# aldma/Bazinga.jl

Hardware: AMD Instinct MI355X
Metric: PANOC inner iterations/sec, n=10^7 l1-quadratic (higher is better)
Workload: dtype f64

## Files before the change

### bazinga.jl_amd/csrc/bz_kernels.h

```cpp
#pragma once
#include <algorithm>
#include <type_traits>

#include <hip/hip_runtime.h>
#include <stdint.h>
#include <math.h>

#include "../../include/bazinga_hip.h"

namespace bz {

constexpr int BLOCK   = 256;
constexpr int WAVES   = BLOCK / 64;
constexpr int PSTRIDE = 2048;

struct ScalarSrc {
    const double* p;
    int count;
    int stride;
};

template <class T> struct PackN;
template <> struct PackN<double> { static constexpr int N = 2; };
template <> struct PackN<float>  { static constexpr int N = 4; };
// ... 2006 lines not shown
                acc[10] = mul_acc(s, nr, acc[10]);
                acc[11] = mul_acc(yy, nr, acc[11]);
            }
        }
        st(x_d, i0, cnt, pxd);
        st(z, i0, cnt, pz);
        st(res, i0, cnt, pr);
        st(s_new, i0, cnt, ps);
        st(y_new, i0, cnt, py);
        if (gx_out) st(gx_out, i0, cnt, pg1);
        if (gz_out) st(gz_out, i0, cnt, pg2);
    });
    block_reduce_store<12>(acc, 1u << 9, parts, slot0);
}

template <class T, int MM> struct CompactVecs {
    const T* S[MM];
    const T* Y[MM];
    int m;
};
struct GateRec {
    unsigned long long w[32];
    unsigned long long seq;
    double val[13];
};
constexpr unsigned long long GATE_ABORT = 1ull << 63;
constexpr unsigned GATE_SPIN_HOST = 2500000u, GATE_SPIN_DEV = 60000000u;

template <int MM> struct CompactCoef {
    double u1[MM];
    double u2h[MM];
    double H0;
    double gam0;
    int uni_rt, trial_rt;
    unsigned long long gate_seq;
    const GateRec* gate_host;
    GateRec* gate_dev;
    int* gate_timeout;
    unsigned gate_spin_host, gate_spin_dev;
};

template <class T, int MM>
__global__ void __launch_bounds__(BLOCK)
k_gram_dots(CompactVecs<T, MM> V, const T* __restrict__ res, int64_t n, double* __restrict__ parts,
            int slot0) {
    double acc[2 * MM];
#pragma unroll
    for (int k = 0; k < 2 * MM; ++k) acc[k] = 0.0;
    bz_for_chunks<T>(n, [&](const int64_t i0, const auto cnt_) {
        const int cnt = cnt_;
        Pack<T> pr = ld(res, i0, cnt);
#pragma unroll
        for (int i = 0; i < MM; ++i) {
            if (i < V.m) {
                Pack<T> ps = ld(V.S[i], i0, cnt), py = ld(V.Y[i], i0, cnt);
#pragma unroll
                for (int e = 0; e < PackN<T>::N; ++e)
                    if (e < cnt) {
                        const T v = T(-1) * pr.v[e];
                        acc[i] = mul_acc(ps.v[e], v, acc[i]);
                        acc[MM + i] = mul_acc(py.v[e], v, acc[MM + i]);
                    }
            }
        }
    });
    block_reduce_store<2 * MM>(acc, 0u, parts, slot0);
// ... 587 lines not shown
                        if ((sq & ~GATE_ABORT) == C.gate_seq) break;
                        __builtin_amdgcn_s_sleep(2);
                        if (++spins > C.gate_spin_dev) { sq = C.gate_seq | GATE_ABORT; *C.gate_timeout = 7; break; }
                    }
                }
                if (lane == 0) gate_sh = sq;
            }
            __syncthreads();
            if (gate_sh & GATE_ABORT) return false;
#pragma unroll
            for (int i = 0; i < MM; ++i) {
                u1[i] = (T)__hip_atomic_load(&C.gate_dev->val[i], __ATOMIC_RELAXED, __HIP_MEMORY_SCOPE_AGENT);
                u2h[i] = (T)__hip_atomic_load(&C.gate_dev->val[5 + i], __ATOMIC_RELAXED, __HIP_MEMORY_SCOPE_AGENT);
            }
            H0 = (T)__hip_atomic_load(&C.gate_dev->val[10], __ATOMIC_RELAXED, __HIP_MEMORY_SCOPE_AGENT);
            z = (T*)(uintptr_t)__double_as_longlong(__hip_atomic_load(&C.gate_dev->val[11], __ATOMIC_RELAXED, __HIP_MEMORY_SCOPE_AGENT));
        }
        }
        return true;
    };
    static_assert(XR == 0 || XR == 2, "XR: stored pairs (0) or iterates with re-evaluated residuals (2)");
    static_assert(XR != 2 || (SPEC && OFF32), "the iterate-history form is pipelined");
    if (SPEC && !OFF32) {
#pragma unroll
        for (int i = 0; i < MM; ++i) { asm volatile("" : "+v"(u1[i])); asm volatile("" : "+v"(u2h[i])); }
        asm volatile("" : "+v"(H0));
        asm volatile("" : "+v"(gl));
        asm volatile("" : "+v"(gamma));
    }
    constexpr bool UDIV = XR == 2 && sizeof(T) == 8;
    T rmu_u = T(0), rgam = T(0);
    if constexpr (UDIV) { rgam = T(1) / gamma; if (uni >= 1) rmu_u = T(1) / P.mu_uniform; }
    const T gam0 = (T)C.gam0, gl0 = gam0 * P.g_lambda;
    constexpr int NS = 10 + 4 * MM + 2;
    double acc[NS];
#pragma unroll
    for (int k = 0; k < NS; ++k) acc[k] = 0.0;
    constexpr bool PIPE = SPEC && OFF32 && XR == 2;
    constexpr int NSTREAMS = MM + 1 + (fam_fk(FAM) ? 2 : 0) + (UNI >= 2 ? 0 : (UNI == 1 ? 1 : 2)) + (TRIAL == 0 ? 0 : 1) +
                             (GKC == FAM_G_L1BOX ? 1 : 0) + (GKC == FAM_G_INDBOX_VEC ? 2 : 0) + (DKC == FAM_D_BOX_VEC ? 2 : 0);
    constexpr int DEPTH = NSTREAMS <= 11 ? 2 : 1;
    constexpr bool NTP = NT && PP == 0;
    struct Stage { Pack<T> q, b, mu, muy, px, ps[MM], xt, gu, glo, ghi, dlo, dhi; };
    using PolQB = std::integral_constant<bool, NTP>;
    using PolNT = std::integral_constant<bool, NT>;
    auto for_fixed_streams = [&](Stage& S, auto&& f) {
        if (fk == BZ_F_DIAG_QUADRATIC) { f(S.q, P.q, PolQB{}); f(S.b, P.b, PolQB{}); }
        if (uni < 1) f(S.mu, P.mu, PolNT{});
        if (uni < 2) f(S.muy, P.muy, PolNT{});
        f(S.px, x, PolNT{});
        if (trial) f(S.xt, (const T*)x_d, PolNT{});
#pragma unroll
        for (int i = 0; i < MM; ++i) f(S.ps[i], V.S[i], PolNT{});
    };
    auto load_stage = [&](Stage& S, unsigned bo) {
        asm volatile("" : "+v"(bo));
        for_fixed_streams(S, [&](Pack<T>& d, const T* p, auto pol) { d = ldo<T, decltype(pol)::value>(p, bo); });
        if constexpr (GKC == FAM_G_L1BOX) S.gu = ldo<T, NT>(P.g_u, bo);
        if constexpr (GKC == FAM_G_INDBOX_VEC) {
            S.glo = P.g_lo_vec ? ldo<T, NT>(P.g_lo_vec, bo) : splat(P.g_lo);
            S.ghi = P.g_hi_vec ? ldo<T, NT>(P.g_hi_vec, bo) : splat(P.g_hi);
        }
        if constexpr (DKC == FAM_D_BOX_VEC) {
            S.dlo = P.D_lo_vec ? ldo<T, NT>(P.D_lo_vec, bo) : splat(P.D_lo);
            S.dhi = P.D_hi_vec ? ldo<T, NT>(P.D_hi_vec, bo) : splat(P.D_hi);
        }
// ... 32 lines not shown
            for (int i = 0; i < MM; ++i) {
                ps[i] = ldo<T, NT>(V.S[i], bo);
                py[i] = ldo<T, NT>(V.Y[i], bo);
            }
        } else {
            if (SPEC && !FAMILY) {
                L.q = ldp<T, NTP>(P.q, i0, cnt); L.b = ldp<T, NTP>(P.b, i0, cnt);
                if (P.uni >= 1) L.mu = splat(P.mu_uniform); else L.mu = ldp<T, NT>(P.mu, i0, cnt);
                if (P.uni >= 2) L.muy = splat(T(0)); else L.muy = ldp<T, NT>(P.muy, i0, cnt);
                L.dlo = splat(P.D_lo); L.dhi = splat(P.D_hi);
                L.gu = splat(T(0)); L.glo = splat(T(0)); L.ghi = splat(T(0));
            } else {
                load_params<T, NT>(P, i0, cnt, L, true, true, true);
                if (FAMILY && uni >= 1) L.mu = splat(P.mu_uniform);
                if (FAMILY && uni >= 2) L.muy = splat(T(0));
            }
            px = ldp<T, NT>(x, i0, cnt);
            if constexpr (XR != 2) prp = ldp<T, NT>(res_prev, i0, cnt);
#pragma unroll
            for (int i = 0; i < MM; ++i)
                if (i < m) {
                    ps[i] = ldp<T, NT>(V.S[i], i0, cnt);
                    if constexpr (XR != 2) py[i] = ldp<T, NT>(V.Y[i], i0, cnt);
                }
        }
        if constexpr (XR == 2) {
            Pack<T> rr[MM + 1];
#pragma unroll
            for (int e = 0; e < N; ++e) {
                if constexpr (UDIV) rmu.v[e] = (uni >= 1) ? rmu_u : T(1) / L.mu.v[e];
#pragma unroll
                for (int i = 0; i <= MM; ++i) {
                    T zz;
                    const T gi = (i == 0) ? gam0 : gamma;
                    const T gli = (i == 0) ? gl0 : gl;
                    rr[i].v[e] = resid_elem<T>(fk, dk, gk, (i < MM) ? ps[i].v[e] : px.v[e], L, e, gi, gli, zz, UDIV,
                                               rmu.v[e], (i < MM) ? ps[i].v[e ^ 1] : px.v[e ^ 1]);
                }
            }
            prp = rr[MM];
#pragma unroll
            for (int i = 0; i < MM; ++i)
#pragma unroll
                for (int e = 0; e < N; ++e) {
                    const T nx = (i + 1 < MM) ? ps[i + 1].v[e] : px.v[e];
                    ps[i].v[e] = nx - ps[i].v[e];
                    py[i].v[e] = rr[i + 1].v[e] - rr[i].v[e];
                }
        }
        if (!trial) compact_d<T, MM>(m, H0, u1, u2h, prp, ps, py, d);
        Pack<T> pxd, pz, pr, pss, pyy, pg1, pgt;
#pragma unroll
        for (int e = 0; e < N; ++e) pxd.v[e] = trial ? pxt.v[e] : px.v[e] + d.v[e];
        T f1[N], p1[N];
#pragma unroll
        for (int e = 0; e < N; ++e) {
            const T xd = pxd.v[e];
            ALOut<T> o1 = al_elem(fk, dk, xd, L.q.v[e], L.b.v[e], L.mu.v[e], L.muy.v[e], L.dlo.v[e], L.dhi.v[e],
                                  pxd.v[e ^ 1] + L.muy.v[e ^ 1], e & 1, UDIV, rmu.v[e]);
            T t = gamma * o1.grad;
            T y = xd - t;
            T zz = prox_elem(gk, y, gl, L.gu.v[e], L.glo.v[e], L.ghi.v[e], pgt.v[e]);
            pz.v[e] = zz; pr.v[e] = xd - zz;
            pg1.v[e] = o1.grad; f1[e] = o1.fterm; p1[e] = o1.pterm;
        }
#pragma unroll
        for (int e = 0; e < N; ++e) {
            const T xd = pxd.v[e], zz = pz.v[e], r = pr.v[e];
            ALOut<T> o2 = al_elem(fk, dk, zz, L.q.v[e], L.b.v[e], L.mu.v[e], L.muy.v[e], L.dlo.v[e], L.dhi.v[e],
                                  pz.v[e ^ 1] + L.muy.v[e ^ 1], e & 1, UDIV, rmu.v[e]);
            T sv = xd - px.v[e];
            T yy = r - prp.v[e];
            T w = UDIV ? div_u(r, gamma, rgam) : r / gamma;
// ... 769 lines not shown
```

### bazinga.jl_amd/csrc/bz_solver.hip

```cpp
#include "bz_solver.h"
#include "bz_spmv.h"
#include "bz_als_dense.h"
#include "bz_csr_host.h"

#include <hip/hip_ext.h>

#include <algorithm>
#include <array>
#include <atomic>
#include <chrono>
#include <cmath>
#include <cstdio>
#include <cstdlib>
#include <cstring>
#include <limits>
#include <optional>
#include <tuple>
#include <type_traits>

namespace bz {

Ctx::~Ctx() {
    for (int r = 0; r < P2P_MAXRANKS; ++r)
        if (mbox_opened[r] && mbox_peer[r]) (void)hipIpcCloseMemHandle(mbox_peer[r]);
// ... 67 lines not shown
    PersistTimeout() : Error(BZ_ERR_HIP, "persistent two-loop kernel: grid barrier timed out (blocks not co-resident?)") {}
};

bool& callback_abort_flag() {
    static thread_local bool flag = false;
    return flag;
}

enum Cat : int { C_TWOLOOP = 0, C_FUSED = 1, C_ALGRAD = 2, C_FB = 3, C_UPDATE = 4,
                 C_COLLECT = 5, C_GATHER = 6, C_MISC = 7, C_DOT = 8, C_GEMV = 9, C_PERSIST = 10, C_GEMV_MFMA = 11, C_FUSED_IT = 12,
                 C_STENCIL_FB = 13, C_STENCIL_UPD = 14, C_XD = 15 };

static int env_int(const char* name, int dflt) { const char* e = std::getenv(name); return e ? std::atoi(e) : dflt; }
static long long env_ll(const char* name, long long dflt) { const char* e = std::getenv(name); return e ? std::atoll(e) : dflt; }
static std::optional<int> env_opt(const char* name) { const char* e = std::getenv(name); return e ? std::optional<int>(std::atoi(e)) : std::nullopt; }
struct CreateKnobs {
    std::optional<int> grid = env_opt("BZ_GRID");
    std::optional<int> persist_blocks = env_opt("BZ_PERSIST_BLOCKS");
    int dense_fused = env_int("BZ_DENSE_FUSED", 1);
    std::optional<int> dense_kp = env_opt("BZ_DENSE_KP");
    std::optional<int> spmv_l = env_opt("BZ_SPMV_L");
    int spq_fused = env_int("BZ_SPQ_FUSED", 1);
    int spls_fused = env_int("BZ_SPLS_FUSED", 1);
    int test_dense_timeout = env_int("BZ_TEST_DENSE_TIMEOUT", 0);
    unsigned dense_spin = (unsigned)env_ll("BZ_DENSE_SPIN", 0);
};
struct BeginKnobs {
    explicit BeginKnobs(int nranks) : gate(env_int("BZ_GATE", nranks > 1 ? 0 : 1)) {}
    int gate;
    int xr = env_int("BZ_XR", 2);
    int skipz = env_int("BZ_SKIPZ", 1);
    int gfc = env_int("BZ_GFC", 0);
    int trialfuse = env_int("BZ_TRIALFUSE", 1);
    int fused_begin = env_int("BZ_FUSED_BEGIN", 1);
    int slackfast = env_int("BZ_SLACKFAST", 1);
    int slackkind = env_int("BZ_SLACKKIND", 1);
    int suc_grid = env_int("BZ_SUC_GRID", 1);
    int stencil_regx = env_int("BZ_STENCIL_REGX", 1);
    int affine_blend = env_int("BZ_AFFINE_BLEND", 1);
    int densesmall = env_int("BZ_DENSESMALL", 1);
    int nt = env_int("BZ_NT", -1);
    int keepp = env_int("BZ_KEEPP", -1);
    int ldsq = env_int("BZ_LDSQ", -1);
    int famrt = env_int("BZ_FAMRT", 0);
    int spec = env_int("BZ_SPEC", 1);
    int xdnt = env_int("BZ_XDNT", 1);
    bool gemv_valu = std::getenv("BZ_GEMV_VALU") != nullptr;
    long long persist_min_n = env_ll("BZ_PERSIST_MIN_N", 300000);
    bool test_persist_timeout = env_int("BZ_TEST_PERSIST_TIMEOUT", 0) != 0;
    int test_gate_timeout = env_int("BZ_TEST_GATE_TIMEOUT", 0);
    unsigned gate_spin = (unsigned)env_ll("BZ_GATE_SPIN", 0);
};
static int read_uni_knob() { return env_int("BZ_UNI", 2); }

template <class F> static void with_bool(bool b, F&& f) { if (b) f(std::true_type{}); else f(std::false_type{}); }
template <class F> static void with_uni(int u, F&& f) {
    if (u >= 2) f(std::integral_constant<int, 2>{});
    else if (u == 1) f(std::integral_constant<int, 1>{});
    else f(std::integral_constant<int, 0>{});
}

template <class T> class Solver final : public SolverBase {
   public:
    Solver(Ctx* c, const bz_problem_desc& d)
        : ctx(c), desc(d), n(d.n), ny(d.ny), nx(d.n), slack(d.slack != 0), env_(c->nranks) {
        if (n <= 0 || ny < 0) throw Error(BZ_ERR_ARG, "n must be positive");
// ... 820 lines not shown
        const T* yv = Y_[state_.lbfgs.spare].p;
        gemv_rows(HB_.p, n, n, yv, (const T*)nullptr, BHy_.p);
        gemv_cols(HB_.p, n, n, sv, b_rpc_, b_nch_, GT_.p, npad);
        {
            ElemParams<T> Pz = P;
            Pz.f_kind = BZ_F_ZERO;
            launch(C_MISC, k_gemv_t_finish<T>, grid, (const T*)GT_.p, b_nch_, npad, sv, Pz, BsH_.p, n, parts_.p, (int)SL_SCRATCH);
        }
        launch(C_MISC, k_dot<T>, grid, (const T*)BHy_.p, sv, T(1), n, parts_.p, (int)SL_AUX);
        launch(C_MISC, k_dot<T>, grid, sv, sv, T(1), n, parts_.p, (int)SL_AUX + 1);
        slot_n[SL_AUX] = slot_n[SL_AUX + 1] = grid;
        gather(SL_AUX, 2, 0u);
        auto v = collect({SL_AUX, SL_AUX + 1}, 0u);
        const T hys = T(v[0]), ss = T(v[1]);
        if (!(ss > T(0))) return;
        const T delta = hys / ss;
        T theta = T(1);
        if (std::abs(delta) < broyden_theta_bar_) {
            const T sg = delta >= T(0) ? T(1) : T(-1);
            theta = (T(1) - sg * broyden_theta_bar_) / (T(1) - delta);
        }
        const T denom = (T(1) / theta - T(1)) * ss + hys;
        if (denom == T(0) || denom != denom) return;
        launch(C_MISC, k_rank1_update<T>, (int)std::min<int64_t>(PSTRIDE, (n * n + BLOCK - 1) / BLOCK), HB_.p, sv,
               (const T*)BHy_.p, (const T*)BsH_.p, T(1) / denom, n);
    }
    bool compact_ok = false;

    struct GatePlan {
        const T* S[CM];
        const T* x;
        T* xd;
        double gam0, gamma;
        int uni, gfc, fam, m_now;
        bool nt, table, keep_params, lds_ring;
        auto key() const { return std::tie(x, xd, gam0, gamma, uni, gfc, fam, m_now, nt, table, keep_params, lds_ring); }
        bool operator==(const GatePlan& o) const { return std::equal(S, S + CM, o.S) && key() == o.key(); }
    };
    static constexpr double KEEP_PARAMS_BYTES = 256e6;
    bool keep_params(bool nt, bool table, int fam) const {
        if (!nt || table || fam != FAM_HEADLINE) return false;
        return env_.keepp >= 0 ? env_.keepp != 0 : (double)n * sizeof(T) * 2 <= KEEP_PARAMS_BYTES;
    }
    bool lds_ring(bool nt, bool table) const { return sizeof(T) == 8 && nt && !table && env_.ldsq != 0; }
    GateRec* gate_host_ = nullptr;
    GateRec* gate_host_dev_ = nullptr;
    DBuf<GateRec> gate_dev_;
    unsigned long long gate_seq_ = 0;
    bool gate_pending_ = false, more_coming_ = false;
    int gate_env_ = 1;
    bool gate_broken_ = false;
    int gate_sabotage_ = 0;
    int64_t n_gate_fallbacks_ = 0;
    GatePlan gate_plan_{};
    double gate_bytes_ = 0.0;
    int64_t n_gated_ = 0, n_gate_aborts_ = 0;
    void gate_alloc() {
        if (gate_host_) return;
        BZ_HIP(hipHostMalloc((void**)&gate_host_, sizeof(GateRec), hipHostMallocMapped));
        std::memset(gate_host_, 0, sizeof(GateRec));
        BZ_HIP(hipHostGetDevicePointer((void**)&gate_host_dev_, gate_host_, 0));
        gate_dev_.alloc(1);
    }
    bool small_vectors() const { return (double)vcap * sizeof(T) < 4.0e9; }
    int xr2_streams(int m_now) const { return (m_now + 1) + pstreams(true, true, true) + 1; }
    bool xr2_plan(int xc_, int m_now, const double* gring, int xr_run, bool zstore, GatePlan& pl) const {
        const int fam = fused_family();
        if (!(env_.xr && small_vectors() && fam >= 0 && xr_run >= m_now)) return false;
        for (int i = 1; i < m_now; ++i)
            if (gring[(xc_ - m_now + i + NXR) % NXR] != (double)state_.gamma) return false;
        std::memset(&pl, 0, sizeof(pl));
        for (int i = 0; i < CM; ++i) {
            const int slot = (xc_ - std::max(0, m_now - i) + NXR) % NXR;
            pl.S[i] = X_[slot].p;
            if (i == 0) pl.gam0 = gring[slot];
        }
        pl.x = X_[xc_].p; pl.xd = X_[(xc_ + 1) % NXR].p;
        pl.gamma = (double)state_.gamma; pl.uni = uni_; pl.fam = fam; pl.m_now = m_now;
        pl.gfc = env_.gfc > 0 ? std::min(grid, env_.gfc * std::max(1, num_cus)) : std::min(grid, std::max(1, num_cus));
        pl.nt = env_.nt >= 0 ? env_.nt != 0 : (double)n * sizeof(T) * (xr2_streams(m_now) + (zstore ? 1 : 0)) > 340e6;
        pl.table = !(env_.spec && fam == FAM_HEADLINE) || env_.famrt;
        pl.keep_params = keep_params(pl.nt, pl.table, fam);
        pl.lds_ring = lds_ring(pl.nt, pl.table);
        return true;
    }
    void launch_xr2(const GatePlan& pl, CompactCoef<CM> C, int trial, T* xd, T* zarg, T* resarg) {
        CompactVecs<T, CM> XV;
        XV.m = CM;
        for (int i = 0; i < CM; ++i) { XV.S[i] = pl.S[i]; XV.Y[i] = nullptr; }
        C.gam0 = pl.gam0;
        const T gam = (T)pl.gamma;
        auto go = [&](auto kernel) {
            launch(C_FUSED_IT, kernel, pl.gfc, XV, C, pl.x, (const T*)nullptr, P, gam, xd, zarg, resarg, (T*)nullptr,
                   (T*)nullptr, n, parts_.p, (int)SL_TRIAL);
        };
        if (pl.table) {
            C.uni_rt = pl.uni; C.trial_rt = trial;
            FusedFn<T> fn = (trial == 0 && !env_.famrt) ? family_kernel<T>(pl.fam, pl.nt, pl.uni) : nullptr;
            const bool ct = fn != nullptr;
            if (!fn) fn = family_kernel<T>(pl.fam, pl.nt, -1);
            if (!fn) throw Error(BZ_ERR_STATE, "no one-pass kernel instantiation for this oracle family");
            form_[C_FUSED_IT] = std::string("k_fused_compact<XR=2,UNI=") + (ct ? std::to_string(pl.uni) : std::string("-1")) + ",NT=" +
                                std::to_string(pl.nt ? 1 : 0) + ",TRIAL=" + (ct ? "0" : "-1") + ",FAM=" + std::to_string(pl.fam) + ">";
            go(fn);
            return;
        }
        form_[C_FUSED_IT] = std::string("k_fused_compact<XR=2,UNI=") + char('0' + pl.uni) + (pl.nt ? ",NT=1" : ",NT=0") +
                            (trial ? ",TRIAL=1" : ",TRIAL=0") + (pl.keep_params ? ",PP=1" : "") + (pl.lds_ring ? ",LQ=1>" : ">");
        with_bool(trial != 0, [&](auto tr) {
            with_uni(pl.uni, [&](auto un) {
                constexpr int TR = decltype(tr)::value, UNI = decltype(un)::value;
                if (pl.lds_ring) {
                    if constexpr (sizeof(T) == 8) {
                        if (pl.keep_params) go(k_fused_compact<T, CM, true, true, true, 2, UNI, TR, FAM_HEADLINE, 1, 1>);
                        else go(k_fused_compact<T, CM, true, true, true, 2, UNI, TR, FAM_HEADLINE, 0, 1>);
                    }
                } else if (pl.nt && pl.keep_params) go(k_fused_compact<T, CM, true, true, true, 2, UNI, TR, FAM_HEADLINE, 1>);
                else if (pl.nt) go(k_fused_compact<T, CM, true, true, true, 2, UNI, TR, FAM_HEADLINE, 0>);
                else go(k_fused_compact<T, CM, false, true, true, 2, UNI, TR, FAM_HEADLINE, 0>);
            });
        });
    }
    void gate_prelaunch(int xd, int m_now) {
        double gr[NXR];
        for (int i = 0; i < NXR; ++i) gr[i] = gring_[i];
        gr[xd] = (double)state_.gamma;
        GatePlan pl;
        if (!xr2_plan(xd, std::min(m_now + 1, state_.lbfgs.M), gr, xr_run_ + 1, false, pl)) return;
        gate_alloc();
        CompactCoef<CM> C2;
        std::memset(&C2, 0, sizeof(C2));
        C2.gate_spin_host = env_.gate_spin ? env_.gate_spin : GATE_SPIN_HOST;
        C2.gate_spin_dev = env_.gate_spin ? 8u * env_.gate_spin : GATE_SPIN_DEV;
        C2.gate_seq = ++gate_seq_; C2.gate_host = gate_host_dev_; C2.gate_dev = gate_dev_.p; C2.gate_timeout = ptimeout_dev_;
        mv(xr2_streams(pl.m_now));
        gate_bytes_ = pending_bytes_;
        launch_xr2(pl, C2, 0, pl.xd, (T*)nullptr, (T*)nullptr);
        gate_plan_ = pl; gate_pending_ = true;
    }
    void gate_release(const CompactCoef<CM>& C, T* zstore) {
        if (gate_sabotage_ > 0 && --gate_sabotage_ == 0) {
// ... 267 lines not shown
        if (!handles) throw Error(BZ_ERR_ARG, "null handles");
        BZ_HIP(hipSetDevice(ctx->device));
        for (int r = 0; r < ctx->nranks; ++r) {
            if (r == ctx->rank) { ar_peer_[r] = ar_local_; continue; }
            if (ar_peer_[r]) continue;
            hipIpcMemHandle_t h;
            std::memcpy(&h, (const char*)handles + (size_t)r * 64, 64);
            BZ_HIP(hipIpcOpenMemHandle(&ar_peer_[r], h, hipIpcMemLazyEnablePeerAccess));
        }
        ar_connected_ = true;
    }
   private:
    const T* allreduce_partials() {
        if (!ar_connected_) throw Error(BZ_ERR_STATE, "row-sharded DenseAffine: bz_problem_allreduce_connect has not been called");
        const unsigned long long seq = ++arseq_;
        const int par = (int)(seq & 1ull);
        VecXchgArgs<T> a;
        std::memset(&a, 0, sizeof(a));
        a.local = JL_.p; a.seq = seq; a.npad = npad; a.nranks = ctx->nranks; a.timeout = ptimeout_dev_;
        for (int r = 0; r < ctx->nranks; ++r) {
            a.peer_slot[r] = ar_slot(ar_peer_[r], par, ctx->rank);
            a.peer_flag[r] = ar_flag(ar_peer_[r], par, ctx->rank);
        }
        a.my_flags = ar_flag(ar_local_, par, 0);
        const int64_t packs = npad / PackN<T>::N;
        const int g = (int)std::max<int64_t>(1, std::min<int64_t>(64, (packs + BLOCK - 1) / BLOCK));
        if (!ar_done_.p) ar_done_.alloc(16);
        ar_done_base_ += (unsigned long long)g;
        a.done = ar_done_.p; a.target = ar_done_base_;
        launch_b(C_GATHER, k_vec_allgather<T>, g, BLOCK, a);
        return ar_slot(ar_local_, par, 0);
    }

    void ensure_z(bool need_res = true) {
        if (state_.z_valid && (state_.res_valid || !need_res)) return;
        if (begin_fb_ok()) {
            mv(1 + pstreams(true, true, true) + 1 + (state_.res_valid ? 0 : 1));
            launch(C_FB, k_zres_elem<T>, grid, (const T*)X_[xc].p, P, state_.gamma, Z_[zc].p,
                   state_.res_valid ? (T*)nullptr : RES_[rc].p, n);
        } else {
            dense_redo([&] {
                algrad(X_[xc].p, D_.p, SL_AUX);
                fbstep(X_[xc].p, D_.p, state_.gamma, Z_[zc].p, state_.res_valid ? (T*)nullptr : RES_[rc].p, SL_ZS);
            });
        }
        state_.z_valid = true; state_.res_valid = true;
    }
    void gather(int first, int cnt, unsigned maxmask, unsigned ymask = 0u) {
        if (!ctx->multi()) return;
        const unsigned keepmask = x_replicated ? ymask : ~0u;
        if (ctx->p2p_on) {
            if (cnt > P2P_PACK) throw Error(BZ_ERR_ARG, "pack too large for the p2p mailbox");
            XchgArgs a;
            std::memset(&a, 0, sizeof(a));
            fill_xchg(a, first, cnt, maxmask);
            a.keepmask = keepmask;
            launch_b(C_GATHER, k_exchange, cnt, 64, a);
            return;
        }
        if (cnt > 32) throw Error(BZ_ERR_ARG, "pack too large");
        SlotCounts counts;
        std::memset(&counts, 0, sizeof(counts));
        for (int i = 0; i < cnt; ++i) counts.set(i, slot_n[first + i]);
        launch_b(C_GATHER, k_pack, cnt, 64, (const double*)parts_.p, counts, first, cnt, maxmask, send_.p, ctx->rank,
                 keepmask);
        BZ_NCCL(ncclAllGather(send_.p + first, recv_.p + (size_t)first * ctx->nranks, cnt, ncclDouble,
                              ctx->comm, ctx->stream));
        for (int s = first; s < first + cnt; ++s) { grp_first[s] = first; grp_cnt[s] = cnt; }
    }
    void fill_xchg(XchgArgs& a, int first, int cnt, unsigned maxmask) {
        a.parts = parts_.p; a.first = first; a.cnt = cnt; a.maxmask = maxmask;
        for (int i = 0; i < cnt; ++i) a.counts.set(i, slot_n[first + i]);
        a.rank = 0; a.nranks = 1;
        if (ctx->p2p_on) {
            a.rank = ctx->rank; a.nranks = ctx->nranks; a.seq = ++ctx->xseq;
            a.recv = recv_.p + (size_t)first * ctx->nranks;
// ... 1086 lines not shown
                BZ_HIP(hipStreamSynchronize(ctx->stream));
                pbase = 0; ctx->pseq = sv_pseq;
                restore();
                persist_ok = false; persist_broken_ = true; ++n_persist_fallbacks_;
                std::fprintf(stderr, "Warning: persistent two-loop kernel timed out at its grid barrier; using the kernel chain\n");
                step_impl();
            }
        } catch (...) {
            more_coming_ = false;
            gate_abort();
            throw;
        }
        if (!more_coming_) gate_abort();
    }
   private:
    std::array<DBuf<T>*, 8> image_bufs() { return {&GX_, &GXN_, &GZ_, &GZN_, &CXS_, &CXD_, &CZS_, &CZN_}; }
    IterState snapshot() {
        IterState sv = state_;
        const auto b = image_bufs();
        for (int i = 0; i < 8; ++i) sv.img[i] = ImageRef{b[i]->p, b[i]->n};
        return sv;
    }
    void put_back(const IterState& sv) {
        state_ = sv;
        const auto b = image_bufs();
        for (int i = 0; i < 8; ++i) { b[i]->p = sv.img[i].p; b[i]->n = sv.img[i].n; }
        cx_keep_ = nullptr;
        state_.gx_valid = aff_track_ && sv.gx_valid; state_.gz_valid = aff_track_ && sv.gz_valid;
    }
    static constexpr int NFC = 10 + 4 * CM + 2;
    static_assert(SL_TRIAL + NFC <= SL_AUX, "k_fused_compact's slots overlap the next group");
    struct Iter {
        T nr0, FBE_x;
        bool stencil_fast_now, use_compact;
        CompactVecs<T, CM> CV;
        CompactCoef<CM> CC;
        TailArgs<T> tail;
        int m_at_trial;
        int xp, xd, xb, rp, rn, zp, zn;
        int xcur, nbt = 0;
        bool have_trial = false, fused_this = false, reset_this = false, sep_trial = false;
        bool img_trial = false;
        bool z_skipped = false, res_skipped = false, gram_from_trial = false;
        bool tail_used = false; unsigned long long tail_ticket = 0;
        bool head_on = false, head_fb = false;
        bool state_imgs = false, halved_here = false;
        bool trial_ok = false; GatePlan trial_plan; CompactCoef<CM> trial_coef;
        double sep_p = 0.0, sep_w = 0.0;
        double gsy[CM] = {0}, gyy[CM] = {0};
        double tp[CM] = {0}, tw[CM] = {0}, tpn = 0.0, twn = 0.0;
        std::vector<double> v;
        bool gen_gram = false;
        int m_gram;
    };
    void step_impl() {
        ++cnt_.k;
        Iter it;
        open_iteration(it);
        if (fused_ok && it.use_compact) trial_onepass(it);
        else if (fused_ok && !slack) trial_sep(it);
        else trial_chain(it);
        step_size_test(it);
        commit(it);
    }
    void open_iteration(Iter& it) {
        it.nr0 = std::sqrt(state_.ss_res);
        it.FBE_x = (state_.f_x - state_.dot_gr + ((alpha / state_.gamma) / T(2)) * (it.nr0 * it.nr0)) + state_.g_z;
        state_.fbe_last = it.FBE_x;
        it.stencil_fast_now = stencil_fast_ && (!ctx->multi() || (ctx->p2p_on && compact_ok));
        it.use_compact = compact_ok && (!state_.lbfgs.order.empty() || (fused_ok && fused_family() >= 0) || it.stencil_fast_now || aff_track_);
        const bool use_persist = persist_ok && !state_.lbfgs.order.empty() && !it.use_compact;
        if (it.use_compact) { it.CV = compact_vecs(); it.CC = compact_prepare(it.CV); std::memset(&it.tail, 0, sizeof(it.tail)); }
        else if (dir_kind_ == BZ_DIR_BROYDEN) { if (!state_.res_valid) ensure_z(); it.tail = broyden_dir(); }
        else it.tail = use_persist ? two_loop_persist() : two_loop();
        it.m_at_trial = it.m_gram = (int)state_.lbfgs.order.size();
        tau = T(1);
        it.xp = xc; it.xd = (xc + 1) % NXR; it.xb = (xc + 2) % NXR;
        it.rp = rc; it.rn = (rc + 1) % NRR; it.zp = zc; it.zn = 1 - zc;
        it.xcur = it.xd;
    }

    void trial_onepass(Iter& it) {
        int gfc = std::min(grid, (env_.gfc > 0 ? env_.gfc : 2) * std::max(1, num_cus));
        const int fam = fused_family();
        const bool headline = env_.spec && fam == FAM_HEADLINE;
        const bool spec = headline && it.CV.m == CM;
        const bool near_stop = (double)stop_norm_ <= 10.0 * opt.tol || (cnt_.k <= 20 && opt.tol > 0.0);
        T* const zstore = (env_.skipz && !near_stop) ? (T*)nullptr : Z_[it.zn].p;
        it.z_skipped = zstore == nullptr;
        const bool small = small_vectors();
        const int m_now = (int)state_.lbfgs.order.size();
        int xr = 0;
        if (env_.xr && small && (fam >= 0 || slack) && xr_run_ >= m_now) {
            xr = 2;
            for (int i = 1; i < m_now; ++i)
                if (gring_[(xc - m_now + i + NXR) % NXR] != (double)state_.gamma) xr = 0;
        }
        if (sy_stale_ && !xr) materialize_pairs();
        if (xr != 2 && !state_.res_valid) ensure_z();
// ... 36 lines not shown
        form_[C_FUSED_IT] = std::string("k_fused_slack_xr") + (snt ? "<NT=1>" : "<NT=0>");
        if (fast) form_[C_FUSED_IT] += hk ? "(fast,l1-box)" : "(fast)";
        auto go = [&](auto kernel) {
            launch(C_FUSED_IT, kernel, gfc, SV, it.CC, P, (const T*)ymul_.p, state_.gamma, X_[it.xd].p, zstore, nx, parts_.p, (int)SL_TRIAL);
        };
        with_bool(snt, [&](auto nt_) {
            constexpr bool NT = decltype(nt_)::value;
            if (fast) {
                with_uni(P.uni, [&](auto un) {
                    constexpr int UNI = decltype(un)::value;
                    if (hk) go(k_fused_slack_xr<T, CM, NT, true, UNI, 1, 1>);
                    else go(k_fused_slack_xr<T, CM, NT, true, UNI, 0, 0>);
                });
            } else if (m_now == CM) go(k_fused_slack_xr<T, CM, NT, true, -1, 0, 0>);
            else go(k_fused_slack_xr<T, CM, NT, false, -1, 0, 0>);
        });
        sy_stale_ = true; it.res_skipped = true;
        it.trial_ok = false;
    }
    void onepass_xr2(Iter& it, T* zstore) {
        GatePlan cur;
        if (!xr2_plan(xc, (int)state_.lbfgs.order.size(), gring_, xr_run_, zstore != nullptr, cur))
            throw Error(BZ_ERR_STATE, "the iterate-history pass does not apply");
        it.CC.gam0 = cur.gam0;
        if (gate_pending_ && cur == gate_plan_) {
            gate_release(it.CC, zstore);
        } else {
            gate_abort();
            mv(xr2_streams(cur.m_now) + (zstore ? 1 : 0));
            launch_xr2(cur, it.CC, 0, cur.xd, zstore, (T*)nullptr);
        }
        sy_stale_ = true; it.res_skipped = true;
        it.trial_ok = env_.trialfuse != 0; it.trial_plan = cur; it.trial_coef = it.CC;
    }
    void onepass_stored(Iter& it, int gfc, T* zstore, bool nt, bool spec, bool off32) {
        if (slack) {
            mv(2 * (2 + 2 * it.CV.m + 4 + (zstore ? 1 : 0)) + pstreams(true, true, true) + (P.uni >= 2 ? 0 : 1), nx);
            form_[C_FUSED] = std::string("k_fused_slack") + (nt ? "<NT=1>" : "<NT=0>");
            with_bool(nt, [&](auto nt_) {
                launch(C_FUSED, k_fused_slack<T, CM, decltype(nt_)::value>, gfc, it.CV, it.CC, (const T*)X_[it.xp].p,
                       (const T*)RES_[it.rp].p, P, (const T*)ymul_.p, state_.gamma, X_[it.xd].p, zstore, RES_[it.rn].p, S_[state_.lbfgs.spare].p,
                       Y_[state_.lbfgs.spare].p, nx, parts_.p, (int)SL_TRIAL);
            });
            return;
        }
        mv(2 + 2 * it.CV.m + pstreams(true, true, true) + 4 + (zstore ? 1 : 0));
        form_[C_FUSED] = std::string("k_fused_compact<XR=0") + (spec ? ",SPEC=1" : ",SPEC=0") + (nt ? ",NT=1>" : ",NT=0>");
        auto go = [&](auto kernel) {
            launch(C_FUSED, kernel, gfc, it.CV, it.CC, (const T*)X_[it.xp].p, (const T*)RES_[it.rp].p, P, state_.gamma, X_[it.xd].p,
                   zstore, RES_[it.rn].p, S_[state_.lbfgs.spare].p, Y_[state_.lbfgs.spare].p, n, parts_.p, (int)SL_TRIAL);
        };
        if (off32 && nt) go(k_fused_compact<T, CM, true, true, true>);
        else if (off32) go(k_fused_compact<T, CM, false, true, true>);
        else if (nt && spec) go(k_fused_compact<T, CM, true, true>);
        else if (nt) go(k_fused_compact<T, CM, true, false>);
        else if (spec) go(k_fused_compact<T, CM, false, true>);
        else go(k_fused_compact<T, CM, false, false>);
    }
    void trial_sep(Iter& it) {
        if (!state_.res_valid) ensure_z();
        for (int k = 0; k < 12; ++k) slot_n[SL_TRIAL + k] = grid;
        mv((it.tail.mode != 2 ? 2 : 1) + 2 + pstreams(true, true, true) + 5);
        form_[C_FUSED] = "k_fused_sep";
        launch(C_FUSED, k_fused_sep<T>, grid, it.tail, (const T*)X_[it.xp].p, (const T*)RES_[it.rp].p, P, state_.gamma,
               X_[it.xd].p, Z_[it.zn].p, RES_[it.rn].p, S_[state_.lbfgs.spare].p, Y_[state_.lbfgs.spare].p, (T*)nullptr, (T*)nullptr, n,
               parts_.p, (int)SL_TRIAL);
// ... 206 lines not shown
                    it.gsy[i] = v[10 + i]; it.gyy[i] = v[10 + CM + i];
                    it.tp[i] = v[10 + 2 * CM + i]; it.tw[i] = v[10 + 3 * CM + i];
                }
                it.tpn = v[10 + 4 * CM]; it.twn = v[10 + 4 * CM + 1];
            } else if (it.have_trial && it.sep_trial) {
                static_assert(SL_TRIAL == SL_FXD && SL_STOP == SL_TRIAL + 9 && SL_GU == SL_TRIAL + 10, "k_fused_sep's slots");
                v = collect_range(SL_TRIAL, 12, 1u << 9);
                it.sep_p = v[10]; it.sep_w = v[11];
                it.gram_from_trial = false;
            } else {
                v = collect({SL_FXD, SL_PXD, SL_GSUM, SL_DOT, SL_SS, SL_FZ, SL_PZ, SL_YS, SL_YTY, SL_STOP},
                            1u << 9);
                it.gram_from_trial = false;
            }
            it.have_trial = false;
            state_.f_x = al_value(v[0], v[1]);
            state_.g_z = g_value(v[2]); state_.dot_gr = T(v[3]); state_.ss_res = T(v[4]);
            const T f_z = al_value(v[5], v[6]);
            state_.fraw_last = f_value(v[5]); state_.f_z_al = f_z;
            const T nr = std::sqrt(state_.ss_res);
            const T f_z_upp = state_.f_x - state_.dot_gr + ((alpha / state_.gamma) / T(2)) * (nr * nr);
            const T tol = T(10) * eps * (T(1) + std::abs(f_z));
            const bool halve = adaptive_ && std::isfinite((double)state_.gamma) && f_z > f_z_upp + tol && state_.gamma >= min_gamma;
            if (halve && it.img_trial) {
                it.img_trial = false; state_.aff_count = 0; ++state_.n_affine_verify;
                cx_keep_ = CXD_.p;
                algrad(X_[it.xcur].p, GX_.p, SL_FXD); ++cnt_.n_grad; state_.gx_valid = true;
                cx_keep_ = nullptr;
                --k;
                continue;
            }
            const T FBE_new = f_z_upp + state_.g_z;
            if (gate_pending_ && !(k == 1 && !halve && (FBE_new <= threshold || k >= max_bt) && T(v[7]) > T(0))) gate_abort();
            if (halve) it.trial_ok = false;
            if (sy_stale_ && !it.trial_ok && (halve || !(FBE_new <= threshold || k >= max_bt))) materialize_pairs();
            if ((!state_.z_valid || !state_.res_valid) && (halve || !(FBE_new <= threshold || k >= max_bt))) ensure_z();
            if (halve) {
                it.halved_here = true;
                state_.gamma = state_.gamma * T(0.5); ++cnt_.n_halv;
                if (state_.gamma < min_gamma)
                    std::fprintf(stderr, "Warning: stepsize `gamma` became too small (%g)\n", (double)state_.gamma);
                sigma = sigma * T(2);
                lbfgs_reset();
                it.fused_this = false; it.reset_this = true;
                continue;
            }
            if (FBE_new <= threshold || k >= max_bt) break;
            tau = (k >= max_bt - 1) ? T(0) : tau / T(2);
            ++it.nbt; ++cnt_.n_bt;
            retrial(it);
        }
    }
    void retrial(Iter& it) {
        const int xb = it.xb;
        mv(3);
        launch(C_MISC, k_blend<T>, grid, (const T*)X_[it.xd].p, (const T*)Z_[it.zp].p, tau, T(1) - tau, X_[xb].p, n);
        it.xcur = xb;
        it.fused_this = false;
        if (it.trial_ok) {
            for (int kk = 0; kk < NFC; ++kk) slot_n[SL_TRIAL + kk] = it.trial_plan.gfc;
            mv(xr2_streams(it.m_at_trial) + 2);
            launch_xr2(it.trial_plan, it.trial_coef, 1, X_[xb].p, Z_[it.zn].p, RES_[it.rn].p);
            onepass_scalars(it, false);
            it.have_trial = true; it.gram_from_trial = true; state_.gx_valid = false; state_.gz_valid = false;
            cnt_.n_grad += 2; cnt_.n_prox += 1;
        } else if (env_.affine_blend && aff_track_ && it.state_imgs && state_.gx_valid && it.nbt == 1 && !it.halved_here && compact_ok &&
                   !generic_ && !ctx->multi() && state_.aff_count + 1 < aff_refresh_) {
            ++state_.aff_count; it.img_trial = true;
            ++state_.n_affine_blends;
            mv(3, ny);
            launch(C_MISC, k_blend<T>, grid_y, (const T*)CXD_.p, (const T*)CZS_.p, tau, T(1) - tau, CZN_.p, ny);
            CXD_.swap(CZN_);
            mv(3);
            launch(C_MISC, k_blend<T>, grid, (const T*)GX_.p, (const T*)GZ_.p, tau, T(1) - tau, GZN_.p, n);
            GX_.swap(GZN_);
            slot_n[SL_FXD] = grid; slot_n[SL_PXD] = grid_y;
            mv(1 + pstreams(true, false, false));
            launch(C_MISC, k_fvalue_elem<T>, grid, (const T*)X_[xb].p, P, n, parts_.p, (int)SL_FXD, (const T*)nullptr);
            mv(2 + pstreams(false, true, false), ny);
            launch(C_MISC, k_yupd<T>, grid_y, (const T*)CXD_.p, P, YU_.p, ny, parts_.p, (int)SL_PXD);
            ++cnt_.n_grad; state_.gx_valid = true;
        } else {
            if (aff_track_) { cx_keep_ = CXD_.p; state_.aff_count = 0; it.img_trial = false; }
            algrad(X_[xb].p, GX_.p, SL_FXD); ++cnt_.n_grad; state_.gx_valid = true;
            cx_keep_ = nullptr;
        }
    }

    void commit(Iter& it) {
        if (aff_track_) {
            GZ_.swap(GZN_);
            CZS_.swap(CZN_);
            CXS_.swap(CXD_);
        }
        const T ys = T(it.v[7]), yty = T(it.v[8]);
        last_ys = ys;
        state_.lbfgs.pw_valid = compact_ok && it.gram_from_trial && (int)state_.lbfgs.order.size() == it.m_gram;
        if (state_.lbfgs.pw_valid) {
            for (int i = 0; i < CM; ++i) { state_.lbfgs.hp[i] = i < it.m_gram ? it.tp[i] : 0.0; state_.lbfgs.hw[i] = i < it.m_gram ? it.tw[i] : 0.0; }
            state_.lbfgs.p_new = it.tpn; state_.lbfgs.w_new = it.twn;
        } else if (compact_ok && it.sep_trial && it.fused_this && it.m_at_trial == 0 && state_.lbfgs.order.empty()) {
            state_.lbfgs.pw_valid = true;
            for (int i = 0; i < CM; ++i) { state_.lbfgs.hp[i] = 0.0; state_.lbfgs.hw[i] = 0.0; }
            state_.lbfgs.p_new = it.sep_p; state_.lbfgs.w_new = it.sep_w;
        }
        if (dir_kind_ == BZ_DIR_BROYDEN) {
            broyden_update();
        } else if (ys > T(0) || dir_kind_ == BZ_DIR_ANDERSON) {
            if (compact_ok && !it.gram_from_trial && !state_.lbfgs.order.empty()) {
                for (int k = 0; k < 2 * CM; ++k) slot_n[SL_GU + k] = grid;
                mv(2 * (int)state_.lbfgs.order.size() + 1);
                launch(C_DOT, k_gram_pair<T, CM>, grid, compact_vecs(), (const T*)Y_[state_.lbfgs.spare].p, n, parts_.p,
                       (int)SL_GU);
                gather(SL_GU, 2 * CM, 0u);
                auto gv = collect_range(SL_GU, 2 * CM, 0u);
                for (int i = 0; i < CM; ++i) { it.gsy[i] = gv[i]; it.gyy[i] = gv[CM + i]; }
            }
            state_.lbfgs.insert(ys, yty, it.gsy, it.gyy, compact_ok, dir_kind_ == BZ_DIR_ANDERSON);
        } else {
            ++cnt_.n_skips;
            materialize_pairs();
// ... 67 lines not shown
```

Measured before the change: 7847.

## Recompute halved-step residual via one-pass iterate-history kernel instead of materializing pairs

When the stepsize is halved during an iteration whose pairs were kept implicit (iterate-history path), the solver no longer materializes the L-BFGS pairs and recomputes z separately. It instead launches the fused XR=2 kernel in a new trial mode 2 with zero L-BFGS coefficients, which takes the residual from the current point (rr[0]) and refreshes z, the residual and the scalars in one pass. This avoids extra full-vector passes on halving events, at the cost of a new kernel mode and more complex state bookkeeping (trial_mode, sy_stale_).

```diff
diff --git a/bazinga.jl_amd/csrc/bz_kernels.h b/bazinga.jl_amd/csrc/bz_kernels.h
--- a/bazinga.jl_amd/csrc/bz_kernels.h
+++ b/bazinga.jl_amd/csrc/bz_kernels.h
@@ -2820,6 +2820,7 @@
                 }
             }
             prp = rr[MM];
+            if (TRIAL != 0 && C.trial_rt == 2) prp = rr[0];
 #pragma unroll
             for (int i = 0; i < MM; ++i)
 #pragma unroll
diff --git a/bazinga.jl_amd/csrc/bz_solver.hip b/bazinga.jl_amd/csrc/bz_solver.hip
--- a/bazinga.jl_amd/csrc/bz_solver.hip
+++ b/bazinga.jl_amd/csrc/bz_solver.hip
@@ -1071,8 +1071,9 @@
             launch(C_FUSED_IT, kernel, pl.gfc, XV, C, pl.x, (const T*)nullptr, P, gam, xd, zarg, resarg, (T*)nullptr,
                    (T*)nullptr, n, parts_.p, (int)SL_TRIAL);
         };
+        C.trial_rt = trial;
         if (pl.table) {
-            C.uni_rt = pl.uni; C.trial_rt = trial;
+            C.uni_rt = pl.uni;
             FusedFn<T> fn = (trial == 0 && !env_.famrt) ? family_kernel<T>(pl.fam, pl.nt, pl.uni) : nullptr;
             const bool ct = fn != nullptr;
             if (!fn) fn = family_kernel<T>(pl.fam, pl.nt, -1);
@@ -2593,6 +2594,7 @@
         bool head_on = false, head_fb = false;
         bool state_imgs = false, halved_here = false;
         bool trial_ok = false; GatePlan trial_plan; CompactCoef<CM> trial_coef;
+        bool xr2_first = false; int trial_mode = 1;
         double sep_p = 0.0, sep_w = 0.0;
         double gsy[CM] = {0}, gyy[CM] = {0};
         double tp[CM] = {0}, tw[CM] = {0}, tpn = 0.0, twn = 0.0;
@@ -2714,6 +2716,7 @@
         }
         sy_stale_ = true; it.res_skipped = true;
         it.trial_ok = env_.trialfuse != 0; it.trial_plan = cur; it.trial_coef = it.CC;
+        it.xr2_first = true;
     }
     void onepass_stored(Iter& it, int gfc, T* zstore, bool nt, bool spec, bool off32) {
         if (slack) {
@@ -2987,7 +2990,8 @@
             const T FBE_new = f_z_upp + state_.g_z;
             if (gate_pending_ && !(k == 1 && !halve && (FBE_new <= threshold || k >= max_bt) && T(v[7]) > T(0))) gate_abort();
             if (halve) it.trial_ok = false;
-            if (sy_stale_ && !it.trial_ok && (halve || !(FBE_new <= threshold || k >= max_bt))) materialize_pairs();
+            const bool halve_xr2 = halve && it.xr2_first && !ctx->multi();
+            if (sy_stale_ && !it.trial_ok && !halve_xr2 && (halve || !(FBE_new <= threshold || k >= max_bt))) materialize_pairs();
             if ((!state_.z_valid || !state_.res_valid) && (halve || !(FBE_new <= threshold || k >= max_bt))) ensure_z();
             if (halve) {
                 it.halved_here = true;
@@ -2997,6 +3001,10 @@
                 sigma = sigma * T(2);
                 lbfgs_reset();
                 it.fused_this = false; it.reset_this = true;
+                if (halve_xr2) {
+                    sy_stale_ = false;
+                    if (env_.trialfuse) retrial_halved(it);
+                }
                 continue;
             }
             if (FBE_new <= threshold || k >= max_bt) break;
@@ -3014,7 +3022,7 @@
         if (it.trial_ok) {
             for (int kk = 0; kk < NFC; ++kk) slot_n[SL_TRIAL + kk] = it.trial_plan.gfc;
             mv(xr2_streams(it.m_at_trial) + 2);
-            launch_xr2(it.trial_plan, it.trial_coef, 1, X_[xb].p, Z_[it.zn].p, RES_[it.rn].p);
+            launch_xr2(it.trial_plan, it.trial_coef, it.trial_mode, X_[xb].p, Z_[it.zn].p, RES_[it.rn].p);
             onepass_scalars(it, false);
             it.have_trial = true; it.gram_from_trial = true; state_.gx_valid = false; state_.gz_valid = false;
             cnt_.n_grad += 2; cnt_.n_prox += 1;
@@ -3041,6 +3049,23 @@
         }
     }
 
+    void retrial_halved(Iter& it) {
+        GatePlan pl;
+        if (!xr2_plan(xc, 0, gring_, 0, true, pl)) throw Error(BZ_ERR_STATE, "the iterate-history pass does not apply");
+        pl.gfc = grid;
+        for (int kk = 0; kk < NFC; ++kk) slot_n[SL_TRIAL + kk] = pl.gfc;
+        CompactCoef<CM> C0;
+        std::memset(&C0, 0, sizeof(C0));
+        mv(xr2_streams(0) + 2);
+        launch_xr2(pl, C0, 2, X_[it.xcur].p, Z_[it.zn].p, RES_[it.rn].p);
+        onepass_scalars(it, false);
+        it.have_trial = true; it.gram_from_trial = true; state_.gx_valid = false; state_.gz_valid = false;
+        it.m_gram = it.m_at_trial = 0;
+        cnt_.n_grad += 1; cnt_.n_prox += 1;
+        sy_stale_ = true;
+        it.trial_ok = true; it.trial_plan = pl; it.trial_coef = C0; it.trial_mode = 2;
+    }
+
     void commit(Iter& it) {
         if (aff_track_) {
             GZ_.swap(GZN_);
```

New measurement: 7749. 1.2% lower.

## Handle stepsize halving with a fused one-pass trial re-evaluation

Applied to the files above, without the earlier changes.

When the trial rejects and gamma is halved, the solver now reruns a single fused iterate-history pass at the new gamma instead of invalidating the trial and running a separate ensure_z plus materialize_pairs. The kernel gains a separate gamx for the current iterate so the residual at x uses the right stepsize. It aims to cut extra kernel launches and memory passes on halving iterations, at the cost of more control logic and a risk of errors in stale-state handling.

```diff
diff --git a/bazinga.jl_amd/csrc/bz_kernels.h b/bazinga.jl_amd/csrc/bz_kernels.h
--- a/bazinga.jl_amd/csrc/bz_kernels.h
+++ b/bazinga.jl_amd/csrc/bz_kernels.h
@@ -2062,6 +2062,7 @@
     double u2h[MM];
     double H0;
     double gam0;
+    double gamx;
     int uni_rt, trial_rt;
     unsigned long long gate_seq;
     const GateRec* gate_host;
@@ -2715,6 +2716,8 @@
     T rmu_u = T(0), rgam = T(0);
     if constexpr (UDIV) { rgam = T(1) / gamma; if (uni >= 1) rmu_u = T(1) / P.mu_uniform; }
     const T gam0 = (T)C.gam0, gl0 = gam0 * P.g_lambda;
+    T gamx = gamma, glx = gl;
+    if constexpr (TRIAL > 0) { gamx = (T)C.gamx; glx = gamx * P.g_lambda; }
     constexpr int NS = 10 + 4 * MM + 2;
     double acc[NS];
 #pragma unroll
@@ -2813,8 +2816,9 @@
 #pragma unroll
                 for (int i = 0; i <= MM; ++i) {
                     T zz;
-                    const T gi = (i == 0) ? gam0 : gamma;
-                    const T gli = (i == 0) ? gl0 : gl;
+                    T gi = (i == 0) ? gam0 : gamma;
+                    T gli = (i == 0) ? gl0 : gl;
+                    if constexpr (TRIAL > 0) { if (i == MM) { gi = gamx; gli = glx; } }
                     rr[i].v[e] = resid_elem<T>(fk, dk, gk, (i < MM) ? ps[i].v[e] : px.v[e], L, e, gi, gli, zz, UDIV,
                                                rmu.v[e], (i < MM) ? ps[i].v[e ^ 1] : px.v[e ^ 1]);
                 }
diff --git a/bazinga.jl_amd/csrc/bz_solver.hip b/bazinga.jl_amd/csrc/bz_solver.hip
--- a/bazinga.jl_amd/csrc/bz_solver.hip
+++ b/bazinga.jl_amd/csrc/bz_solver.hip
@@ -123,6 +123,7 @@
     int skipz = env_int("BZ_SKIPZ", 1);
     int gfc = env_int("BZ_GFC", 0);
     int trialfuse = env_int("BZ_TRIALFUSE", 1);
+    int nonplain = env_int("BZ_NONPLAIN", 1);
     int fused_begin = env_int("BZ_FUSED_BEGIN", 1);
     int slackfast = env_int("BZ_SLACKFAST", 1);
     int slackkind = env_int("BZ_SLACKKIND", 1);
@@ -1009,6 +1010,7 @@
         const T* x;
         T* xd;
         double gam0, gamma;
+        double gamx;
         int uni, gfc, fam, m_now;
         bool nt, table, keep_params, lds_ring;
         auto key() const { return std::tie(x, xd, gam0, gamma, uni, gfc, fam, m_now, nt, table, keep_params, lds_ring); }
@@ -1052,6 +1054,7 @@
             pl.S[i] = X_[slot].p;
             if (i == 0) pl.gam0 = gring[slot];
         }
+        pl.gamx = gring[xc_];
         pl.x = X_[xc_].p; pl.xd = X_[(xc_ + 1) % NXR].p;
         pl.gamma = (double)state_.gamma; pl.uni = uni_; pl.fam = fam; pl.m_now = m_now;
         pl.gfc = env_.gfc > 0 ? std::min(grid, env_.gfc * std::max(1, num_cus)) : std::min(grid, std::max(1, num_cus));
@@ -1065,7 +1068,7 @@
         CompactVecs<T, CM> XV;
         XV.m = CM;
         for (int i = 0; i < CM; ++i) { XV.S[i] = pl.S[i]; XV.Y[i] = nullptr; }
-        C.gam0 = pl.gam0;
+        C.gam0 = pl.gam0; C.gamx = pl.gamx;
         const T gam = (T)pl.gamma;
         auto go = [&](auto kernel) {
             launch(C_FUSED_IT, kernel, pl.gfc, XV, C, pl.x, (const T*)nullptr, P, gam, xd, zarg, resarg, (T*)nullptr,
@@ -1084,6 +1087,7 @@
         }
         form_[C_FUSED_IT] = std::string("k_fused_compact<XR=2,UNI=") + char('0' + pl.uni) + (pl.nt ? ",NT=1" : ",NT=0") +
                             (trial ? ",TRIAL=1" : ",TRIAL=0") + (pl.keep_params ? ",PP=1" : "") + (pl.lds_ring ? ",LQ=1>" : ">");
+        if (trial && pl.gamx != pl.gamma) form_[C_FUSED_IT] += "(halved)";
         with_bool(trial != 0, [&](auto tr) {
             with_uni(pl.uni, [&](auto un) {
                 constexpr int TR = decltype(tr)::value, UNI = decltype(un)::value;
@@ -1417,16 +1421,17 @@
         return ar_slot(ar_local_, par, 0);
     }
 
-    void ensure_z(bool need_res = true) {
+    void ensure_z(bool need_res = true) { ensure_z(need_res, state_.gamma); }
+    void ensure_z(bool need_res, T gam) {
         if (state_.z_valid && (state_.res_valid || !need_res)) return;
         if (begin_fb_ok()) {
             mv(1 + pstreams(true, true, true) + 1 + (state_.res_valid ? 0 : 1));
-            launch(C_FB, k_zres_elem<T>, grid, (const T*)X_[xc].p, P, state_.gamma, Z_[zc].p,
+            launch(C_FB, k_zres_elem<T>, grid, (const T*)X_[xc].p, P, gam, Z_[zc].p,
                    state_.res_valid ? (T*)nullptr : RES_[rc].p, n);
         } else {
             dense_redo([&] {
                 algrad(X_[xc].p, D_.p, SL_AUX);
-                fbstep(X_[xc].p, D_.p, state_.gamma, Z_[zc].p, state_.res_valid ? (T*)nullptr : RES_[rc].p, SL_ZS);
+                fbstep(X_[xc].p, D_.p, gam, Z_[zc].p, state_.res_valid ? (T*)nullptr : RES_[rc].p, SL_ZS);
             });
         }
         state_.z_valid = true; state_.res_valid = true;
@@ -2579,6 +2584,7 @@
     static_assert(SL_TRIAL + NFC <= SL_AUX, "k_fused_compact's slots overlap the next group");
     struct Iter {
         T nr0, FBE_x;
+        T gam_state;
         bool stencil_fast_now, use_compact;
         CompactVecs<T, CM> CV;
         CompactCoef<CM> CC;
@@ -2612,6 +2618,7 @@
     }
     void open_iteration(Iter& it) {
         it.nr0 = std::sqrt(state_.ss_res);
+        it.gam_state = state_.gamma;
         it.FBE_x = (state_.f_x - state_.dot_gr + ((alpha / state_.gamma) / T(2)) * (it.nr0 * it.nr0)) + state_.g_z;
         state_.fbe_last = it.FBE_x;
         it.stencil_fast_now = stencil_fast_ && (!ctx->multi() || (ctx->p2p_on && compact_ok));
@@ -2986,9 +2993,11 @@
             }
             const T FBE_new = f_z_upp + state_.g_z;
             if (gate_pending_ && !(k == 1 && !halve && (FBE_new <= threshold || k >= max_bt) && T(v[7]) > T(0))) gate_abort();
-            if (halve) it.trial_ok = false;
-            if (sy_stale_ && !it.trial_ok && (halve || !(FBE_new <= threshold || k >= max_bt))) materialize_pairs();
-            if ((!state_.z_valid || !state_.res_valid) && (halve || !(FBE_new <= threshold || k >= max_bt))) ensure_z();
+            const bool halve_onepass = halve && halved_onepass_ok(it);
+            const bool rejected = halve || !(FBE_new <= threshold || k >= max_bt);
+            if (halve && !halve_onepass) it.trial_ok = false;
+            if (sy_stale_ && !it.trial_ok && rejected && !(halve && env_.nonplain && !slack)) materialize_pairs();
+            if ((!state_.z_valid || !state_.res_valid) && rejected && !halve_onepass) ensure_z(true, it.gam_state);
             if (halve) {
                 it.halved_here = true;
                 state_.gamma = state_.gamma * T(0.5); ++cnt_.n_halv;
@@ -2996,7 +3005,9 @@
                     std::fprintf(stderr, "Warning: stepsize `gamma` became too small (%g)\n", (double)state_.gamma);
                 sigma = sigma * T(2);
                 lbfgs_reset();
+                sy_stale_ = false;
                 it.fused_this = false; it.reset_this = true;
+                if (halve_onepass) halved_trial_onepass(it);
                 continue;
             }
             if (FBE_new <= threshold || k >= max_bt) break;
@@ -3004,6 +3015,23 @@
             ++it.nbt; ++cnt_.n_bt;
             retrial(it);
         }
+    }
+    bool halved_onepass_ok(const Iter& it) const {
+        return env_.nonplain && it.trial_ok && !it.trial_plan.table && !slack;
+    }
+    void halved_trial_onepass(Iter& it) {
+        GatePlan pl;
+        if (!xr2_plan(xc, 0, gring_, xr_run_, true, pl)) throw Error(BZ_ERR_STATE, "the iterate-history pass does not apply");
+        pl.gfc = grid;
+        std::memset(&it.trial_coef, 0, sizeof(it.trial_coef));
+        it.trial_plan = pl; it.m_at_trial = it.m_gram = 0;
+        for (int kk = 0; kk < NFC; ++kk) slot_n[SL_TRIAL + kk] = pl.gfc;
+        mv(xr2_streams(0) + 2);
+        launch_xr2(pl, it.trial_coef, 1, X_[it.xcur].p, Z_[it.zn].p, RES_[it.rn].p);
+        onepass_scalars(it, false);
+        sy_stale_ = true;
+        it.have_trial = true; it.gram_from_trial = true; state_.gx_valid = false; state_.gz_valid = false;
+        cnt_.n_grad += 1; cnt_.n_prox += 1;
     }
     void retrial(Iter& it) {
         const int xb = it.xb;
```

After: 7682 before, 7805 after (median of 5 runs). Within noise of the previous version (+1.6%).
